# talmolab/sleap-nn

Hardware: AMD Instinct MI355X
Metric: frames/sec bottom-up UNet 1024x1024 inference (higher is better)
Workload: dtype f32

## Files before the change

sleap_nn_amd/csrc/model.hip:

```cpp
#include <algorithm>
#include <atomic>
#include <cmath>
#include <cstring>
#include <mutex>
#include <type_traits>
#include <vector>

#include "model_internal.h"
#include "train_kernels.h"

namespace ph {

static thread_local std::string g_err;

void set_error(const char* fmt, ...) {
  char buf[1024];
  va_list ap;
  va_start(ap, fmt);
  vsnprintf(buf, sizeof(buf), fmt, ap);
  va_end(ap);
  g_err = buf;
}

}
// ... 353 lines not shown
        if (!widx_ok(d.weight) || !widx_ok(d.bias)) return fail("weight index out of range", i);
        if (weight_numel[d.bias] != d.cout) return fail("bias size mismatch", i);
        if (d.kind == PH_OP_CONVT && d.ksize != 3) return fail("transposed conv: only kernel 3 (stride 2, padding 1, output padding 1)", i);
        if (d.ksize != 3) {
          if (!(d.ksize & 1) || d.ksize < 1 || d.ksize > 9) return fail("kernel_size must be odd and <= 9", i);
          if (weight_numel[d.weight] != (int64_t)(d.cin0 + d.cin1) * d.cout * d.ksize * d.ksize) return fail("weight size mismatch", i);
          const int coutp_k = pad16(d.cout);
          op.bn_g = gemm_choose_bn(coutp_k);
          auto pack_k = [&](const auto* w, auto& out) { pack_gemm(w, d.cout, d.cin0, d.cin1, d.ksize * d.ksize, op.bn_g, out); };
          ok = pack_upload(m, pack_k, weights[d.weight], index_array(d.weight), &op.w_gemm_dev) == PH_OK &&
               pack_upload(m, pad_vec((size_t)((coutp_k + op.bn_g - 1) / op.bn_g) * op.bn_g, d.cout), weights[d.bias], index_array(d.bias), &op.b_gemm_dev) == PH_OK;
          if (ok && d.kind == PH_OP_CONV) {
            const int cin_total = d.cin0 + d.cin1;
            const int parts[2] = {d.cin0, d.cin1}, offs[2] = {0, d.cin0};
            int max_bn = 32;
            const std::vector<double> iwk = index_array(d.weight);
            for (int part = 0; part < 2 && ok; ++part) {
              if (parts[part] <= 0) continue;
              op.bn_dk[part] = gemm_choose_bn(pad16(parts[part]));
              max_bn = std::max(max_bn, op.bn_dk[part]);
              auto pack_dk = [&](const auto* w, auto& out) {
                std::remove_reference_t<decltype(out)> dw;
                dgrad_weight(w, d.cout, cin_total, offs[part], parts[part], dw, d.ksize);
                pack_gemm(dw.data(), parts[part], d.cout, 0, d.ksize * d.ksize, op.bn_dk[part], out);
              };
              ok = pack_upload(m, pack_dk, weights[d.weight], iwk, &op.wdk_gemm_dev[part]) == PH_OK;
            }
            if (ok) {
              std::vector<float> zb((size_t)pad16(std::max(d.cin0, d.cin1)) + 2 * max_bn, 0.f);
              ok = upload(m, zb, &op.zero_bias_dev) == PH_OK;
            }
          }
          break;
        }
        if (d.kind == PH_OP_CONVT && d.cin1 != 0) return fail("transposed conv takes one source", i);
        if (weight_numel[d.weight] != (int64_t)(d.cin0 + d.cin1) * d.cout * 9) return fail("weight size mismatch", i);
        const int coutp = pad16(d.cout);
        op.bn = choose_bn(coutp);
        const bool tr = d.kind == PH_OP_CONVT;
        const std::vector<double> iw = index_array(d.weight), ib = index_array(d.bias);
        auto pack_reg = [&](const auto* w, auto& out) { pack_conv(w, tr, d.cin0, d.cin1, d.cout, op.bn, out); };
        auto pack_dma = [&](const auto* w, auto& out) {
          std::remove_reference_t<decltype(out)> tmp;
          pack_conv(w, tr, d.cin0, d.cin1, d.cout, op.bn, tmp);
          repack_dma(tmp, op.bn, out);
        };
        ok = pack_upload(m, pack_reg, weights[d.weight], iw, &op.w_dev) == PH_OK && pack_upload(m, pack_dma, weights[d.weight], iw, &op.w_dma_dev) == PH_OK &&
             pack_upload(m, pad_vec((size_t)((coutp + op.bn - 1) / op.bn) * op.bn, d.cout), weights[d.bias], ib, &op.b_dev) == PH_OK;
        auto derive_wino = [&](const float* src, int cin_a, int cin_b, int cout_, int bn, float** dst) {
          if (bn != 64 && bn != 32) return true;
          const int panels = ((pad16(cout_) + bn - 1) / bn) * (pad16(cin_a) / 16 + (cin_b > 0 ? pad16(cin_b) / 16 : 0));
          float* w = nullptr;
          if (hipMalloc(&w, (size_t)wino_pack_floats(panels, bn) * sizeof(float)) != hipSuccess) return false;
          m->allocs.push_back(w);
          if (launch_wino_pack(src, w, panels, bn, nullptr) != PH_OK) return false;
          add_derived(m, DERIVED_WINO, src, w, panels, bn);
          *dst = w;
          return true;
        };
        if (ok && !tr) ok = derive_wino(op.w_dev, d.cin0, d.cin1, d.cout, op.bn, &op.w_wino_dev);
        auto derive_wino2 = [&](const float* src, int cin_a, int cin_b, int cout_, int bn, float** dst) {
          if (bn != 64) return true;
          const int panels = ((pad16(cout_) + 63) / 64) * (pad16(cin_a) / 16 + (cin_b > 0 ? pad16(cin_b) / 16 : 0));
          float* w = nullptr;
          if (hipMalloc(&w, (size_t)wino2d_pack_floats(panels, 64) * sizeof(float)) != hipSuccess) return false;
          m->allocs.push_back(w);
          if (launch_wino2d_pack(src, w, panels, 64, nullptr) != PH_OK) return false;
          add_derived(m, DERIVED_WINO2D, src, w, panels, 64);
          *dst = w;
          return true;
        };
        if (ok && !tr) ok = derive_wino2(op.w_dev, d.cin0, d.cin1, d.cout, op.bn, &op.w_wino2_dev);
        if (ok && !tr && op.bn == 32 && coutp == 32 && pad16(d.cin0) + (d.cin1 > 0 ? pad16(d.cin1) : 0) >= 64) {
          auto pack_64 = [&](const auto* w, auto& out) { pack_conv(w, false, d.cin0, d.cin1, d.cout, 64, out); };
          ok = pack_upload(m, pack_64, weights[d.weight], iw, &op.w_n64_dev) == PH_OK && pack_upload(m, pad_vec(64, d.cout), weights[d.bias], ib, &op.b_n64_dev) == PH_OK &&
               derive_wino2(op.w_n64_dev, d.cin0, d.cin1, d.cout, 64, &op.w_wino2_dev);
        }
        auto derive_wino4 = [&](const float* src, int cin_a, int cin_b, int cout_, int bn, float** dst) {
          if (bn != 64 || pad16(cin_a) + (cin_b > 0 ? pad16(cin_b) : 0) < 64) return true;
          const int ntiles = (pad16(cout_) + 63) / 64, nchunks = pad16(cin_a) / 16 + (cin_b > 0 ? pad16(cin_b) / 16 : 0);
          float* w = nullptr;
          if (hipMalloc(&w, (size_t)wino4_pack_floats(ntiles, nchunks) * sizeof(float)) != hipSuccess) return false;
          m->allocs.push_back(w);
          if (launch_wino4_pack(src, w, ntiles, nchunks, nullptr) != PH_OK) return false;
          add_derived(m, DERIVED_WINO4, src, w, ntiles, nchunks);
          *dst = w;
          return true;
        };
        if (ok && !tr) ok = derive_wino4(op.w_dev, d.cin0, d.cin1, d.cout, op.bn, &op.w_wino4_dev);
        if (ok && !tr && op.w_n64_dev) ok = derive_wino4(op.w_n64_dev, d.cin0, d.cin1, d.cout, 64, &op.w_wino4_dev);
        auto derive_w16 = [&](const float* src, int cin_, int cout_, int bn, float** dst, int cin_b = 0) {
          const int cip = pad16(cin_), cibp = cin_b > 0 ? pad16(cin_b) : 0, cop = pad16(cout_);
          if (bn != 32 || !w16_shape_ok(cip, cibp, cop)) return true;
          const int chunks = (cip + cibp) / 16, nbs = cop / 16;
          float* w = nullptr;
          if (hipMalloc(&w, (size_t)w16_pack_floats(chunks, nbs) * sizeof(float)) != hipSuccess) return false;
          m->allocs.push_back(w);
          if (launch_w16_pack(src, w, chunks, nbs, nullptr) != PH_OK) return false;
          add_derived(m, DERIVED_W16, src, w, chunks, nbs);
          *dst = w;
          return true;
        };
        if (ok && !tr) ok = derive_w16(op.w_dev, d.cin0, d.cout, op.bn, &op.w_w16_dev, d.cin1);
        if (ok && !tr) {
          const int nblocks = coutp / 16, chunks16 = pad16(d.cin0) / 16 + (d.cin1 > 0 ? pad16(d.cin1) / 16 : 0);
          float* w = nullptr;
          ok = hipMalloc(&w, (size_t)sm_pack_floats(nblocks, chunks16) * sizeof(float)) == hipSuccess;
          if (ok) {
            m->allocs.push_back(w);
            ok = launch_sm_pack(op.w_dev, w, nblocks, chunks16, op.bn, nullptr) == PH_OK;
            add_derived(m, DERIVED_SMALLMAP, op.w_dev, w, nblocks, chunks16).n_tiles = op.bn;
            op.w_sm_dev = w;
          }
        }
        if (ok && !tr) {
          op.bn_g = gemm_choose_bn(coutp);
          auto pack_g = [&](const auto* w, auto& out) { pack_gemm(w, d.cout, d.cin0, d.cin1, 9, op.bn_g, out); };
          ok = pack_upload(m, pack_g, weights[d.weight], iw, &op.w_gemm_dev) == PH_OK &&
               pack_upload(m, pad_vec((size_t)((coutp + op.bn_g - 1) / op.bn_g) * op.bn_g, d.cout), weights[d.bias], ib, &op.b_gemm_dev) == PH_OK;
        }
        const bool c16 = d.kind == PH_OP_CONV && d.cin1 == 0 && d.cin0 <= 16 && d.cout <= 16;
        if (ok && c16) {
          auto pack_16 = [&](const auto* w, auto& out) { pack_c16(w, d.cout, d.cin0, out); };
          auto pack_16d = [&](const auto* w, auto& out) {
            std::remove_reference_t<decltype(out)> dw;
            dgrad_weight(w, d.cout, d.cin0, 0, d.cin0, dw);
            pack_c16(dw.data(), d.cin0, d.cout, out);
          };
          ok = pack_upload(m, pack_16, weights[d.weight], iw, &op.w16_dev) == PH_OK && pack_upload(m, pack_16d, weights[d.weight], iw, &op.wd16_dev) == PH_OK;
        }
        if (ok && tr) {
          op.bn_t = gemm_choose_bn(coutp);
          const size_t npad_t = (size_t)((coutp + op.bn_t - 1) / op.bn_t) * op.bn_t;
          for (int ph = 0; ph < 4 && ok; ++ph) {
            const int py = ph >> 1, px = ph & 1, nt = (1 + py) * (1 + px);
            auto pack_p = [&](const auto* w, auto& out) {
              std::remove_reference_t<decltype(out)> wp((size_t)d.cout * d.cin0 * nt);
              for (int t = 0; t < nt; ++t) {
                const int ty = px ? t >> 1 : t, tx = px ? t & 1 : 0;
                const int ky = py ? 2 * ty : 1, kx = px ? 2 * tx : 1;
                for (int co = 0; co < d.cout; ++co)
                  for (int ci = 0; ci < d.cin0; ++ci) wp[((size_t)co * d.cin0 + ci) * nt + t] = w[(((size_t)ci * d.cout + co) * 3 + ky) * 3 + kx];
              }
              pack_gemm(wp.data(), d.cout, d.cin0, 0, nt, op.bn_t, out);
            };
            ok = pack_upload(m, pack_p, weights[d.weight], iw, &op.wt_phase_dev[ph]) == PH_OK;
          }
          if (ok) ok = pack_upload(m, pad_vec(npad_t, d.cout), weights[d.bias], ib, &op.bt_dev) == PH_OK;
          if (ok && d.weight2 >= 0) {
            if (!widx_ok(d.weight2) || !widx_ok(d.bias2) || weight_numel[d.weight2] != d.cout || weight_numel[d.bias2] != d.cout) return fail("transposed conv: scale / shift must be (cout)", i);
            ok = pack_upload(m, pad_vec(npad_t, d.cout), weights[d.weight2], index_array(d.weight2), &op.wt_scale_dev) == PH_OK &&
                 pack_upload(m, pad_vec(npad_t, d.cout), weights[d.bias2], index_array(d.bias2), &op.wt_shift_dev) == PH_OK;
          }
          if (ok) {
            const int cinp = pad16(d.cin0);
            op.bn_td = gemm_choose_bn(cinp);
            auto pack_dg = [&](const auto* w, auto& out) { pack_gemm(w, d.cin0, d.cout, 0, 9, op.bn_td, out); };
            std::vector<float> zb((size_t)cinp + 128, 0.f);
            ok = pack_upload(m, pack_dg, weights[d.weight], iw, &op.wt_dgrad_dev) == PH_OK && upload(m, zb, &op.zero_bias_dev) == PH_OK;
          }
        }
        if (ok && d.kind == PH_OP_CONV) {
          const int cin_total = d.cin0 + d.cin1;
          const int parts[2] = {d.cin0, d.cin1}, offs[2] = {0, d.cin0};
          int max_bn = 32;
          for (int part = 0; part < 2 && ok; ++part) {
            if (parts[part] <= 0) continue;
            op.bn_d[part] = choose_bn(pad16(parts[part]));
// ... 414 lines not shown
```

sleap_nn_amd/csrc/net_kernels.h:

```cpp
#pragma once
#include <hip/hip_runtime.h>

#include <algorithm>
#include <cstdint>

namespace ph {

struct ConvArgs {
  const float* src0;
  const float* src1;
  const float* wpack;
  const float* bias;
  float* dst;
  int c0p, c1p, coutp;
  int B, H, W;
  int relu;
  int bn;
  unsigned long long* clock_probe = nullptr;
  const float* wpack_dma = nullptr;
  const float* zeros = nullptr;
  int accumulate = 0;
  int dma_stagger = 1;
  const float* wpack_wino = nullptr;
  const float* wpack_wino2 = nullptr;
// ... 143 lines not shown
  int sh = 0, sw = 0;
};
int64_t window_attn_bwd_scratch_floats(int B, int H, int W, int C, int heads, int w);
int launch_window_attn_bwd(const WindowAttnBwdArgs& a, hipStream_t s);
int launch_patch_merge_gather(const float* src, float* dst, int B, int H, int W, int c, hipStream_t s);
int launch_patch_merge_scatter(const float* gsrc, float* gdst, int accumulate, int B, int H, int W, int c, hipStream_t s);
int launch_grad_fanout(const float* gy, float* gx, int accumulate, size_t n, hipStream_t s);
int launch_scale_samples(const float* src, const float* scale, float* dst, size_t per_sample, int B, hipStream_t s);
int launch_scale_samples_add(float* dst, const float* res, const float* scale, size_t per_sample, int B, hipStream_t s);
int launch_vec_add(float* dst, const float* src, int n, hipStream_t s);
int launch_patch_merge_ln(const float* src, const float* gamma, const float* beta, float* dst, int B, int H, int W, int c, float eps, hipStream_t s);
struct WindowAttnF16Args {
  const void* qkv = nullptr;
  const float* table = nullptr;
  const float* qkv_bias = nullptr;
  void* dst = nullptr;
  int B = 0, H = 0, W = 0, C = 0, heads = 0;
  int w = 0;
  int sh = 0, sw = 0;
};
int launch_window_attn_f16(const WindowAttnF16Args& a, hipStream_t s);
int launch_patch_merge_ln_f16(const void* src, const float* gamma, const float* beta, void* dst, int B, int H, int W, int c, float eps, hipStream_t s);
int launch_gemm(const GemmArgs& a, hipStream_t s);
int launch_patch_stem_norm(const PatchStemArgs& a, hipStream_t s);
struct GrnArgs {
  const float* src = nullptr;
  const float* weight = nullptr;
  const float* bias = nullptr;
  float* dst = nullptr;
  float* partial = nullptr;
  int B = 0, HW = 0, c = 0, cp = 0;
};
int grn_slices(int HW);
int grn_slice_pixels(int HW);
int64_t grn_scratch_floats(int B, int HW, int cp);
int launch_grn(const GrnArgs& a, hipStream_t s);
int grn_fused_nseg(int HW);
int64_t grn_fused_partial_floats(int M, int HW, int cp);
int launch_grn_finalize(const float* partial, const float* weight, float* scale, int B, int HW, int c, int cp, hipStream_t s);
int launch_grn_fold_bias(const float* w2, const float* b2, const float* grn_bias, float* dst, int cout, int cin, hipStream_t s);
int64_t gemm_pack_floats(int coutp, int c0p, int bn);
int launch_grn_scale_weights(const float* wpack, const float* scale, float* dst, int B, int coutp, int c0p, int bn, hipStream_t s);
struct MlpArgs {
  const float* x = nullptr;
  const float* w1img = nullptr;
  const float* w2img = nullptr;
  const float* b1 = nullptr;
  const float* b2 = nullptr;
  const float* scale = nullptr;
  const float* residual = nullptr;
  float* dst = nullptr;
  int M = 0, C = 0;
};
bool cnblock_mlp_fits(int c, int cp, int hidden);
int launch_cnblock_mlp(const MlpArgs& a, hipStream_t s);
int gemm_choose_bn(int coutp);
int prepare_convnext_kernels();
int launch_stem(const StemArgs& a, hipStream_t s);
int prepare_kernels();
int conv_lds_bytes(int bn);
int launch_conv3x3(const ConvArgs& a, hipStream_t s);
int launch_wino_pack(const float* wpack, float* wino, int panels, int bn, hipStream_t s);
int64_t wino_pack_floats(int panels, int bn);
struct PackSegment {
  const float* src;
  float* dst;
  unsigned long long total;
  int bn;
  unsigned first_block;
};
int launch_wino_pack_multi(const PackSegment* seg_dev, int n_seg, unsigned total_blocks, hipStream_t s);
int launch_wino2d_pack_multi(const PackSegment* seg_dev, int n_seg, unsigned total_blocks, hipStream_t s);
int launch_stem_wino_pack(const float* w1, float* w1w, hipStream_t s);
int launch_stem_wino2d_pack(const float* w1, float* w2, hipStream_t s);
int launch_conv3x3_dma(const ConvArgs& a, hipStream_t s);
bool conv3x3_dma_honours_mask(const ConvArgs& a);
bool conv3x3_dma_is_f2x2(const ConvArgs& a);
bool conv3x3_dma_is_wino2d(const ConvArgs& a);
bool conv3x3_dma_is_w16_head(const ConvArgs& a);
int conv3x3_dma_variant(const ConvArgs& a);
int launch_wino2d_pack(const float* wpack, float* wino, int panels, int bn, hipStream_t s);
int64_t wino2d_pack_floats(int panels, int bn);
int launch_conv3x3_wino2d(const ConvArgs& a, hipStream_t s);
int launch_wino4_pack(const float* wpack, float* wino, int ntiles, int nchunks, hipStream_t s);
int64_t wino4_pack_floats(int ntiles, int nchunks);
int launch_conv3x3_wino4(const ConvArgs& a, hipStream_t s);
bool wino4_fits(const ConvArgs& a);
bool conv3x3_dma_is_wino4(const ConvArgs& a);
int prepare_wino4_kernels();
bool wino2d_fits(const ConvArgs& a);
int wino2d_ksplit(const ConvArgs& a);
int launch_splitk_reduce(const float* part, long long stride, int ks, const float* bias, float* dst, float* dst_pool, int B, int H, int W, int coutp, int relu, hipStream_t s);
int wino4_ksplit_shape(int B, int H, int W, int cinp, int coutp, int splitk, int n_cu);
int64_t wino4_split_scratch_bytes(int B, int H, int W, int cinp, int coutp, int splitk, int n_cu);
int wino2d_ksplit_shape(int B, int H, int W, int cinp, int coutp, int splitk, int n_cu);
int64_t wino2d_split_scratch_bytes(int B, int H, int W, int cinp, int coutp, int splitk, int n_cu);
int prepare_wino2d_kernels();
int launch_w16_pack(const float* wpack, float* w16, int chunks, int nbs, hipStream_t s);
int64_t w16_pack_floats(int chunks, int nbs);
int launch_conv3x3_w16(const ConvArgs& a, hipStream_t s);
bool w16_fits(const ConvArgs& a);
bool w16_takes_head(const ConvArgs& a);
bool w16_shape_ok(int c0p, int c1p, int coutp);
int prepare_w16_kernels();
int launch_sm_pack(const float* wpack, float* dst, int nblocks, int chunks16, int bn, hipStream_t s);
int64_t sm_pack_floats(int nblocks, int chunks16);
int launch_conv3x3_sm(const ConvArgs& a, hipStream_t s);
bool sm_fits(const ConvArgs& a);
double sm_cost_us(const ConvArgs& a, int n_cu);
bool conv3x3_takes_sm(const ConvArgs& a);
int launch_input_conv(const InputConvArgs& a, hipStream_t s);
int launch_pool(const float* src, float* dst, int B, int H, int W, int cp, hipStream_t s);
int launch_upsample(const float* src, float* dst, int B, int H, int W, int cp, hipStream_t s);
int launch_zero_stuff(const float* src, float* dst, int B, int H, int W, int cp, hipStream_t s);
int launch_global_maxpool(const float* src, float* dst, int B, int HW, int cp, hipStream_t s);
int launch_softmax_rows(float* x, int rows, int n, hipStream_t s);
int launch_nhwc_to_nchw(const float* src, float* dst, int B, int HW, int cp, int c, hipStream_t s);

}
```

sleap_nn_amd/csrc/wino4_kernels.hip:

```cpp
#include <type_traits>

#include "common.h"
#include "net_kernels.h"

#ifndef W4_EXP
#define W4_EXP 0
#endif

namespace ph {

typedef float f32x16 __attribute__((ext_vector_type(16)));
typedef float f32x4 __attribute__((ext_vector_type(4)));
typedef float f32x2 __attribute__((ext_vector_type(2)));

constexpr int W4_TX = 8, W4_TY = 4;
constexpr int W4_PW = 4 * W4_TX;
constexpr int W4_PH = 4 * W4_TY;
constexpr int W4_RAW_PITCH = 36;
constexpr int W4_RAW_PLANE = 688;
constexpr int W4_RAW_FLOATS = 3072;
static_assert(W4_RAW_PITCH >= W4_PW + 2 && W4_RAW_PITCH % 4 == 0, "a halo row fits its pitch and starts 16-byte aligned");
static_assert(W4_RAW_PLANE >= (W4_PH + 3) * W4_RAW_PITCH && W4_RAW_PLANE % 64 % 32 == 16, "a plane holds 18 halo rows + the overshoot row; planes 16 banks apart (mod 32): conflict-free ds_read_b128");
static_assert(4 * W4_RAW_PLANE <= W4_RAW_FLOATS, "four planes fit a raw slot");
constexpr int W4_V_FLOATS = 36 * 128;
constexpr int W4_LDS_FLOATS = 36 * 1024;
constexpr int W4_Q_FLOATS = 36 * 64 * 4;
constexpr int P4_WAVE_FLOATS = 4 * 256 + 128;

__device__ __forceinline__ float wino4_g_row(int k, float g0, float g1, float g2) {
  switch (k) {
    case 0: return 0.25f * g0;
    case 1: return (-1.f / 6.f) * ((g0 + g2) + g1);
    case 2: return (-1.f / 6.f) * ((g0 + g2) - g1);
    case 3: return (1.f / 24.f) * g0 + ((1.f / 12.f) * g1 + (1.f / 6.f) * g2);
    case 4: return (1.f / 24.f) * g0 + ((-1.f / 12.f) * g1 + (1.f / 6.f) * g2);
    default: return g2;
  }
}
__global__ __launch_bounds__(256) void wino4_pack_kernel(const float* __restrict__ src, float* __restrict__ dst, int ntiles, int nchunks) {
  __shared__ float unit[W4_Q_FLOATS];
  const int quarter = blockIdx.x % (4 * nchunks), ntile = blockIdx.x / (4 * nchunks);
  const int tid = threadIdx.x;
  const int row = tid >> 2, kcl = tid & 3;
  const int nt = row >> 5, lx = row & 31, lh = kcl >> 1, j = kcl & 1;
  const float* w = src + (((size_t)ntile * nchunks + (quarter >> 2)) * 9 * 64 + row) * 16 + (quarter & 3) * 4 + kcl;
  const size_t ts = (size_t)64 * 16;
  float g[9];
#pragma unroll
  for (int t = 0; t < 9; ++t) g[t] = w[t * ts];
#pragma unroll
  for (int xi = 0; xi < 6; ++xi) {
    float h[3];
#pragma unroll
    for (int kx = 0; kx < 3; ++kx) h[kx] = wino4_g_row(xi, g[0 * 3 + kx], g[1 * 3 + kx], g[2 * 3 + kx]);
#pragma unroll
    for (int nu = 0; nu < 6; ++nu) {
      const float u = wino4_g_row(nu, h[0], h[1], h[2]);
      const int p = xi * 6 + nu, pgp = p / 9, pl = p % 9;
      unit[(nt * 4 + pgp) * P4_WAVE_FLOATS + (pl < 8 ? (((pl >> 1) * 64 + lh * 32 + lx) << 2) + j * 2 + (pl & 1) : 1024 + ((lh * 32 + lx) << 1) + j)] = u;
    }
  }
  __syncthreads();
  float* out = dst + (size_t)blockIdx.x * W4_Q_FLOATS;
#pragma unroll 4
  for (int i = tid; i < W4_Q_FLOATS; i += 256) out[i] = unit[i];
}
int64_t wino4_pack_floats(int ntiles, int nchunks) { return (int64_t)ntiles * 4 * nchunks * W4_Q_FLOATS; }
int launch_wino4_pack(const float* wpack, float* wino, int ntiles, int nchunks, hipStream_t s) {
  hipLaunchKernelGGL(wino4_pack_kernel, dim3((unsigned)(ntiles * 4 * nchunks)), dim3(256), 0, s, wpack, wino, ntiles, nchunks);
  PH_HIP_CHECK(hipGetLastError());
  return PH_OK;
}

__device__ __forceinline__ void w4_deal_tile(int id, int tiles, int nt_count, int rot, int* tile, int* ntile) {
  if ((tiles & 7) == 0) {
    const int xcd = id & 7, j = id >> 3;
    *ntile = (j % nt_count + rot) % nt_count;
    *tile = xcd * (tiles >> 3) + j / nt_count;
  } else {
    *ntile = (id % nt_count + rot) % nt_count;
    *tile = id / nt_count;
  }
}

__device__ __forceinline__ void w4_col_pass(const float (&t)[6], float (&v)[6]) {
  const float a = fmaf(-4.f, t[2], t[4]);
  const float b = fmaf(-4.f, t[1], t[3]);
  const float c = t[4] - t[2];
  const float d0 = t[3] - t[1];
  const float d = d0 + d0;
  v[0] = fmaf(4.f, t[0], fmaf(-5.f, t[2], t[4]));
  v[1] = a + b;
  v[2] = a - b;
  v[3] = c + d;
  v[4] = c - d;
  v[5] = fmaf(4.f, t[1], fmaf(-5.f, t[3], t[5]));
}

template <int P, int N>
__device__ __forceinline__ void p4_vput(float* slot, int vwq, int vwd, const float* v) {
  if constexpr (N > 0) {
    constexpr int pgc = P / 9, pl = P % 9;
    if constexpr (pl == 8) {
      slot[pgc * P4_WAVE_FLOATS + vwd] = v[0];
      p4_vput<P + 1, N - 1>(slot, vwq, vwd, v + 1);
    } else if constexpr ((pl & 1) == 0 && N >= 2) {
      *reinterpret_cast<float2*>(slot + pgc * P4_WAVE_FLOATS + (pl >> 1) * 256 + vwq) = make_float2(v[0], v[1]);
      p4_vput<P + 2, N - 2>(slot, vwq, vwd, v + 2);
    } else {
      slot[pgc * P4_WAVE_FLOATS + (pl >> 1) * 256 + vwq + (pl & 1)] = v[0];
      p4_vput<P + 1, N - 1>(slot, vwq, vwd, v + 1);
    }
  }
}

template <bool LOWRES, bool KS = false>
__global__ __launch_bounds__(512) void conv3x3_wino4_kernel(ConvArgs a) {
  extern __shared__ __attribute__((aligned(16))) float lds[];
  const int tid = threadIdx.x;
  const int lane = tid & 63;
  const int pw = __builtin_amdgcn_readfirstlane(tid >> 6);
  const int nt = pw >> 2, pg = pw & 3;
  const int lx = lane & 31, lh = lane >> 5;
  const int xg = pw < 4 ? (pw >> 1) : 2 + ((pw - 4) >> 1);
  const int typ = 2 * (pw & 1) + (lane >> 5), txp = (lane >> 2) & 7, cp = lane & 3;

  const int tiles_x = (a.W + W4_PW - 1) / W4_PW;
  const int tiles_y = (a.H + W4_PH - 1) / W4_PH;
  const int tiles = tiles_x * tiles_y * a.B;
  const int ntc = (a.coutp + 63) / 64;
  const int units = tiles * ntc;
  const int total = KS ? units * a.ksplit : units;
  const int Q0 = a.c0p / 4, Q1 = a.c1p / 4, Q = Q0 + Q1;
  constexpr int lowres = LOWRES ? 1 : 0;
  const int Hl = a.H >> 1, Wl = a.W >> 1;

#ifdef W4_CLOCK
  const unsigned long long clk_c0 = __builtin_amdgcn_s_memtime(), clk_r0 = __builtin_amdgcn_s_memrealtime();
#endif
  float* const rawbuf = lds;
  float* const vbuf = lds + 2 * W4_RAW_FLOATS;

  const float alpha = xg == 0 ? -4.f : -1.f, beta = xg == 0 ? 1.f : 2.f, nbeta = -beta;
  const int pbase_f = cp * W4_RAW_PLANE + (4 * typ + (xg == 2 ? 0 : 1)) * W4_RAW_PITCH + 4 * txp;
  const int pbase_l = cp * W4_RAW_PLANE + (2 * typ) * W4_RAW_PITCH + 2 * txp;
  const int lhy = (pw * 64 + lane) / (W4_PW + 2), lhx = (pw * 64 + lane) - lhy * (W4_PW + 2);
  const int lwr = lhy * W4_RAW_PITCH + lhx;
  const int vwq = ((cp >> 1) * 32 + typ * 8 + txp) * 4 + (cp & 1) * 2;
  const int vwd = 1024 + ((cp >> 1) * 32 + typ * 8 + txp) * 2 + (cp & 1);
  const int vrq = pg * P4_WAVE_FLOATS + lane * 4, vrd = pg * P4_WAVE_FLOATS + 1024 + lane * 2;

  struct Plan {
    int b, x0, y0, ntile;
  };
  const int G = (int)gridDim.x;
  const bool rotate = (a.coutp & 63) != 0 && (a.coutp & 63) <= 32 && ntc > 1 && (((tiles & 7) == 0) ? ((G & 7) == 0 && (G >> 3) % ntc == 0) : (G % ntc == 0));
  auto setup = [&](int vid, Plan& P) {
    int t, ntile;
    w4_deal_tile(vid, tiles, ntc, rotate ? vid / G : 0, &t, &ntile);
    const int tx = t % tiles_x;
    t /= tiles_x;
    const int ty = t % tiles_y;
    P.b = t / tiles_y;
    P.x0 = tx * W4_PW;
    P.y0 = ty * W4_PH;
    P.ntile = ntile;
  };

  const __amdgpu_buffer_rsrc_t wrsrc = __builtin_amdgcn_make_buffer_rsrc((void*)a.wpack_wino4, 0, (int)((unsigned)ntc * (unsigned)Q * (unsigned)(W4_Q_FLOATS * 4)), 0x00020000);
  const unsigned w_lane = (unsigned)(pw * P4_WAVE_FLOATS + lane * 4) * 4u;
  const unsigned w_lane9 = (unsigned)(pw * P4_WAVE_FLOATS + 1024 + lane * 2) * 4u;

  for (int vid = blockIdx.x; vid < total; vid += gridDim.x) {
#ifdef W4_STAMP
    const unsigned long long tile_t0 = __builtin_amdgcn_s_memtime();
#endif
    Plan P;
    const int ksl = KS ? vid / units : 0;
    const int qbeg = KS ? ksl * Q / a.ksplit : 0;
    const int qend = KS ? (ksl + 1) * Q / a.ksplit : Q;
    setup(KS ? vid - ksl * units : vid, P);
    unsigned off0[2], off1[2];
#pragma unroll
    for (int i = 0; i < 2; ++i) {
      const int hy = lhy + 15 * i, hx = lhx;
      const int gy = P.y0 + hy - 1, gx = P.x0 + hx - 1;
      const bool in = (i == 0 || pw < 2) && hy < W4_PH + 2 && gy >= 0 && gy < a.H && gx >= 0 && gx < a.W;
      off0[i] = in ? (unsigned)((P.b * a.H + gy) * a.W + gx) * (unsigned)(a.c0p * 4) : 0xFFFFFF00u;
      if (!lowres) {
        off1[i] = (in && a.c1p > 0) ? (unsigned)((P.b * a.H + gy) * a.W + gx) * (unsigned)(a.c1p * 4) : 0xFFFFFF00u;
      } else {
        const int sy = min(max((P.y0 >> 1) - 1 + hy, 0), Hl - 1), sx = min(max((P.x0 >> 1) - 1 + hx, 0), Wl - 1);
        off1[i] = (hy < W4_PH / 2 + 2 && hx < W4_PW / 2 + 2) ? (unsigned)((P.b * Hl + sy) * Wl + sx) * (unsigned)(a.c1p * 4) : 0xFFFFFF00u;
      }
    }
    const __amdgpu_buffer_rsrc_t rsrc0 = __builtin_amdgcn_make_buffer_rsrc((void*)a.src0, 0, (int)((unsigned)(a.B * a.H * a.W) * (unsigned)(a.c0p * 4)), 0x00020000);
// ... 269 lines not shown
        P4_SB
        P4_ST(1)
        if constexpr (MM) {
          acc[8] = P4_MFMA(wf9[0], vf9.x, acc[8]);
          vf0 = *reinterpret_cast<const f32x4*>(vq);
          acc[6] = P4_MFMA(wf[3][2], vf3[2], acc[6]);
        }
        P4_SB
        load_raw(q + 3);
        P4_SB
        P4_ST(2)
        if constexpr (MM) {
          acc[7] = P4_MFMA(wf[3][3], vf3[3], acc[7]);
          load_w(q, 3);
          vf1 = *reinterpret_cast<const f32x4*>(vq + 256);
          P4_ST(3)
          acc[8] = P4_MFMA(wf9[1], vf9.y, acc[8]);
          load_w(q, 4);
        }
        t_rows(xg_tag, lr_tag, 0);
        t_read(xg_tag, lr_tag, raw, 1);
        P4_SB
        P4_ST(4)
        if constexpr (MM) {
          acc[0] = P4_MFMA(wf[0][0], vf0[0], acc[0]);
          acc[1] = P4_MFMA(wf[0][1], vf0[1], acc[1]);
          vf2 = *reinterpret_cast<const f32x4*>(vq + 512);
          acc[0] = P4_MFMA(wf[0][2], vf0[2], acc[0]);
          acc[1] = P4_MFMA(wf[0][3], vf0[3], acc[1]);
          load_w(q + 1, 0);
        }
        t_rows(xg_tag, lr_tag, 1);
        P4_SB
        P4_ST(5)
        if constexpr (MM) {
          acc[2] = P4_MFMA(wf[1][0], vf1[0], acc[2]);
          acc[3] = P4_MFMA(wf[1][1], vf1[1], acc[3]);
          vf3 = *reinterpret_cast<const f32x4*>(vq + 768);
        }
        t_cols(xg_tag, lr_tag, first, vslot);
        if constexpr (MM) {
          acc[2] = P4_MFMA(wf[1][2], vf1[2], acc[2]);
          acc[3] = P4_MFMA(wf[1][3], vf1[3], acc[3]);
          load_w(q + 1, 1);
        }
        P4_SB
        P4_ST(6)
        if constexpr (MM) {
          acc[4] = P4_MFMA(wf[2][0], vf2[0], acc[4]);
          acc[5] = P4_MFMA(wf[2][1], vf2[1], acc[5]);
          vf9 = *reinterpret_cast<const float2*>(vd);
        }
        if constexpr (PAIR) t_cols(xg_tag, lr_tag, second, vslot);
        if constexpr (MM) {
          acc[4] = P4_MFMA(wf[2][2], vf2[2], acc[4]);
          acc[5] = P4_MFMA(wf[2][3], vf2[3], acc[5]);
          load_w(q + 1, 2);
        }
        P4_SB
        P4_ST(7)
        asm volatile("s_waitcnt lgkmcnt(0)" ::: "memory");
        if (!(W4_EXP & 4)) __builtin_amdgcn_s_barrier();
        P4_SB
        P4_ST_END
      }
    };
    auto run = [&](auto xg_tag, auto mm_tag) __attribute__((always_inline)) {
      if constexpr (LOWRES) {
        const int qs = min(max(Q0 - 1, qbeg), qend);
        quarters(xg_tag, mm_tag, std::false_type{}, qbeg, qs);
        quarters(xg_tag, mm_tag, std::true_type{}, qs, qend);
      } else {
        quarters(xg_tag, mm_tag, std::false_type{}, qbeg, qend);
      }
    };
    auto run_mm = [&](auto mm_tag) __attribute__((always_inline)) {
      switch (xg) {
        case 0: run(std::integral_constant<int, 0>{}, mm_tag); break;
        case 1: run(std::integral_constant<int, 1>{}, mm_tag); break;
        case 2: run(std::integral_constant<int, 2>{}, mm_tag); break;
        default: run(std::integral_constant<int, 3>{}, mm_tag); break;
      }
    };
    if (nt == 1 && P.ntile * 64 + 32 >= a.coutp) {
      run_mm(std::false_type{});
    } else {
      run_mm(std::true_type{});
      acc[6] = P4_MFMA(wf[3][0], vf3[0], acc[6]);
      acc[7] = P4_MFMA(wf[3][1], vf3[1], acc[7]);
      acc[8] = P4_MFMA(wf9[0], vf9.x, acc[8]);
      acc[6] = P4_MFMA(wf[3][2], vf3[2], acc[6]);
      acc[7] = P4_MFMA(wf[3][3], vf3[3], acc[7]);
      acc[8] = P4_MFMA(wf9[1], vf9.y, acc[8]);
    }

#ifdef W4_STAMP
    const unsigned long long tile_t2 = __builtin_amdgcn_s_memtime();
#endif
    float* const exch = lds;
    auto dump = [&](int r) __attribute__((always_inline)) {
      int d0 = ((pg * 9 * 32 + lx) * 8 + ((nt * 4 + lh) ^ (lx & 7))) << 2;
      asm volatile("" : "+v"(d0));
#pragma unroll
      for (int kk = 0; kk < 2; ++kk) {
        float* const dk = exch + (d0 ^ (kk << 3));
#pragma unroll
        for (int i = 0; i < 9; ++i) {
          f32x4 v;
          if (r == 0) {
            v[0] = acc[i][4 * kk + 0];
            v[1] = acc[i][4 * kk + 1];
            v[2] = acc[i][4 * kk + 2];
            v[3] = acc[i][4 * kk + 3];
          } else {
            v[0] = acc[i][8 + 4 * kk + 0];
            v[1] = acc[i][8 + 4 * kk + 1];
            v[2] = acc[i][8 + 4 * kk + 2];
            v[3] = acc[i][8 + 4 * kk + 3];
          }
          *reinterpret_cast<f32x4*>(dk + i * 1024) = v;
        }
      }
      asm volatile("s_waitcnt lgkmcnt(0)" ::: "memory");
    };
    auto finish = [&](int round) __attribute__((always_inline)) {
      const int tile = tid >> 4, cq = (tid >> 1) & 7, hc = tid & 1;
      const int ty = tile >> 3, tx = tile & 7;
      int z0 = ((tile * 8 + (cq ^ (tile & 7))) << 2) + 2 * hc;
      asm volatile("" : "+v"(z0));
      const float* zp = exch + z0;
      f32x2 z[4][6];
#pragma unroll
      for (int n = 0; n < 6; ++n) {
        f32x2 m[6];
#pragma unroll
        for (int x = 0; x < 6; ++x) m[x] = *reinterpret_cast<const f32x2*>(zp + (x * 6 + n) * 1024);
#pragma unroll
        for (int e = 0; e < 2; ++e) {
          const float s12 = m[1][e] + m[2][e], d12 = m[1][e] - m[2][e], s34 = m[3][e] + m[4][e], d34 = m[3][e] - m[4][e];
          z[0][n][e] = (m[0][e] + s12) + s34;
          z[1][n][e] = fmaf(2.f, d34, d12);
          z[2][n][e] = fmaf(4.f, s34, s12);
          z[3][n][e] = fmaf(8.f, d34, d12) + m[5][e];
        }
      }
      const int co = P.ntile * 64 + (cq >> 2) * 32 + round * 16 + (cq & 3) * 4 + 2 * hc;
      const f32x2 bias = KS ? f32x2{0.f, 0.f} : *reinterpret_cast<const f32x2*>(a.bias + co);
      const int oy0 = P.y0 + 4 * ty, ox = P.x0 + 4 * tx;
      const bool live = oy0 < a.H && ox < a.W && co < a.coutp;
      f32x2 prow[2];
#pragma unroll
      for (int aa = 0; aa < 4; ++aa) {
        const f32x2 s12 = z[aa][1] + z[aa][2], d12 = z[aa][1] - z[aa][2], s34 = z[aa][3] + z[aa][4], d34 = z[aa][3] - z[aa][4];
        f32x2 y[4];
        y[0] = ((z[aa][0] + s12) + s34) + bias;
        y[1] = (d12 + 2.f * d34) + bias;
        y[2] = (s12 + 4.f * s34) + bias;
        y[3] = ((d12 + 8.f * d34) + z[aa][5]) + bias;
        if (live) {
          float* const dp = a.dst + ((size_t)(P.b * a.H + oy0 + aa) * a.W + ox) * a.coutp + co + (KS ? (size_t)ksl * a.split_stride : (size_t)0);
#pragma unroll
          for (int bb = 0; bb < 4; ++bb) {
            f32x2 v = y[bb];
            if (a.relu) {
#pragma unroll
              for (int e = 0; e < 2; ++e) v[e] = fmaxf(v[e], 0.f);
            }
            if (a.relu_mask_src) {
              const f32x2 f = *reinterpret_cast<const f32x2*>(a.relu_mask_src + (dp - a.dst) + (size_t)bb * a.coutp);
#pragma unroll
              for (int e = 0; e < 2; ++e) v[e] = f[e] > 0.f ? v[e] : 0.f;
            }
            y[bb] = v;
            if ((KS || !a.skip_dst) && !(W4_EXP & 512)) *reinterpret_cast<f32x2*>(dp + (size_t)bb * a.coutp) = v;
          }
          if (!KS && a.dst_pool) {
            f32x2 m0, m1;
#pragma unroll
            for (int e = 0; e < 2; ++e) {
              m0[e] = fmaxf(y[0][e], y[1][e]);
              m1[e] = fmaxf(y[2][e], y[3][e]);
            }
            if (aa & 1) {
#pragma unroll
              for (int e = 0; e < 2; ++e) {
                m0[e] = fmaxf(m0[e], prow[0][e]);
                m1[e] = fmaxf(m1[e], prow[1][e]);
              }
              float* const pp = a.dst_pool + ((size_t)(P.b * (a.H >> 1) + ((oy0 + aa) >> 1)) * (a.W >> 1) + (ox >> 1)) * a.coutp + co;
              *reinterpret_cast<f32x2*>(pp) = m0;
              *reinterpret_cast<f32x2*>(pp + a.coutp) = m1;
            } else {
              prow[0] = m0;
              prow[1] = m1;
            }
          }
        }
      }
      asm volatile("s_waitcnt lgkmcnt(0)" ::: "memory");
    };
#ifdef W4_STAMP
    unsigned long long e1 = 0, e2 = 0, e3 = 0;
#define P4_ET(x) x = __builtin_amdgcn_s_memtime();
#else
#define P4_ET(x)
#endif
    dump(0);
    __builtin_amdgcn_s_barrier();
    P4_ET(e1)
    finish(0);
    __builtin_amdgcn_s_barrier();
    P4_ET(e2)
    dump(1);
    __builtin_amdgcn_s_barrier();
    P4_ET(e3)
    finish(1);
    __builtin_amdgcn_s_barrier();
#ifdef W4_STAMP
    if (a.clock_probe && lane == 0 && vid == (int)blockIdx.x) {
      unsigned long long* o = a.clock_probe + ((size_t)blockIdx.x * 12 + pw) * 8;
#ifdef W4_STTILE
      o[0] = (tile_t1 - tile_t0) * (unsigned long long)(qend - qbeg);
      o[1] = st[0] + st[1] + st[2] + st[3] + st[4] + st[5] + st[6] + st[7];
      o[2] = (e1 - tile_t2) * (unsigned long long)(qend - qbeg);
      o[3] = (e2 - e1) * (unsigned long long)(qend - qbeg);
      o[4] = (e3 - e2) * (unsigned long long)(qend - qbeg);
      o[5] = (__builtin_amdgcn_s_memtime() - e3) * (unsigned long long)(qend - qbeg);
      o[6] = o[7] = 0;
#else
#pragma unroll
      for (int i = 0; i < 8; ++i) o[i] = st[i];
#endif
    }
#endif
  }
#ifdef W4_CLOCK
  if (a.clock_probe && tid == 0) {
    a.clock_probe[blockIdx.x * 2] = __builtin_amdgcn_s_memtime() - clk_c0;
    a.clock_probe[blockIdx.x * 2 + 1] = __builtin_amdgcn_s_memrealtime() - clk_r0;
  }
#endif
}

int prepare_wino4_kernels() {
  hipError_t e = hipSuccess;
  if (e == hipSuccess) e = hipFuncSetAttribute(reinterpret_cast<const void*>(conv3x3_wino4_kernel<false, false>), hipFuncAttributeMaxDynamicSharedMemorySize, W4_LDS_FLOATS * (int)sizeof(float));
  if (e == hipSuccess) e = hipFuncSetAttribute(reinterpret_cast<const void*>(conv3x3_wino4_kernel<true, false>), hipFuncAttributeMaxDynamicSharedMemorySize, W4_LDS_FLOATS * (int)sizeof(float));
  if (e == hipSuccess) e = hipFuncSetAttribute(reinterpret_cast<const void*>(conv3x3_wino4_kernel<false, true>), hipFuncAttributeMaxDynamicSharedMemorySize, W4_LDS_FLOATS * (int)sizeof(float));
  if (e == hipSuccess) e = hipFuncSetAttribute(reinterpret_cast<const void*>(conv3x3_wino4_kernel<true, true>), hipFuncAttributeMaxDynamicSharedMemorySize, W4_LDS_FLOATS * (int)sizeof(float));
  if (e != hipSuccess) {
    set_error("hipFuncSetAttribute(wino4) failed: %s", hipGetErrorString(e));
    return PH_E_HIP;
  }
  return PH_OK;
}

bool wino4_fits(const ConvArgs& a) {
  if (!a.wpack_wino4 || a.bn != 64 || (a.H & 3) || (a.W & 3) || a.head_w || a.accumulate) return false;
  if (a.src1_lowres && (!a.src1 || (a.H & 1) || (a.W & 1))) return false;
  const uint64_t px = (uint64_t)a.B * a.H * a.W;
  if (px * (uint64_t)a.c0p * 4 >= 0xFFFFFF00ull || px * (uint64_t)a.c1p * 4 >= 0xFFFFFF00ull || px >= 0x7FFFFFFFull) return false;
  const uint64_t wbytes = (uint64_t)((a.coutp + 63) / 64) * (uint64_t)((a.c0p + a.c1p) / 4) * W4_Q_FLOATS * 4;
  if (wbytes >= 0xFFFFFF00ull) return false;
  if (a.use_wino4 >= 2) return true;
  int n_cu = 0;
  if (device_cu_count(&n_cu) != PH_OK || n_cu <= 0) n_cu = 256;
  const bool may_split = a.split_scratch != nullptr;
  const int ks4 = may_split ? wino4_ksplit_shape(a.B, a.H, a.W, a.c0p + a.c1p, a.coutp, a.splitk, n_cu) : 1;
  const int ks2 = may_split ? wino2d_ksplit_shape(a.B, a.H, a.W, a.c0p + a.c1p, a.coutp, a.splitk, n_cu) : 1;
  const long ntc = (a.coutp + 63) / 64;
  const long t4 = (long)((a.H + W4_PH - 1) / W4_PH) * ((a.W + W4_PW - 1) / W4_PW) * a.B * ntc;
  const long t2 = (long)((a.H + 15) / 16) * ((a.W + 15) / 16) * a.B * ntc;
  const double Qn = (a.c0p + a.c1p) / 4.0;
  const double cost4 = (double)((t4 * ks4 + n_cu - 1) / n_cu) * (11.0 + 1.5 * Qn / ks4) + (ks4 > 1 ? 8.0 : 0.0);
  const double cost2 = (double)((t2 * ks2 + n_cu - 1) / n_cu) * (8.0 + 1.0 * Qn / ks2) + (ks2 > 1 ? 8.0 : 0.0);
  return cost4 <= cost2;
}
// ... 56 lines not shown
```

Before: 3036.

## Widen wino4 epilogue stores to 16 bytes via DPP lane pair trade

The Winograd F(4,3) epilogue used to write 8-byte float2 values per output pixel. Adjacent lanes now swap halves with DPP cndmask, so each lane holds four channels for one pixel and issues 16-byte stores with an sc1 cache policy. Pooled outputs get the same treatment. To keep channels contiguous, the weight pack and the channel mapping change for full tiles, and ReLU is hoisted ahead of the trade. This adds inline-asm DPP work, and the weight layout and epilogue mapping must stay consistent.

```diff
diff --git a/sleap_nn_amd/csrc/model.hip b/sleap_nn_amd/csrc/model.hip
--- a/sleap_nn_amd/csrc/model.hip
+++ b/sleap_nn_amd/csrc/model.hip
@@ -459,8 +459,8 @@
           float* w = nullptr;
           if (hipMalloc(&w, (size_t)wino4_pack_floats(ntiles, nchunks) * sizeof(float)) != hipSuccess) return false;
           m->allocs.push_back(w);
-          if (launch_wino4_pack(src, w, ntiles, nchunks, nullptr) != PH_OK) return false;
-          add_derived(m, DERIVED_WINO4, src, w, ntiles, nchunks);
+          if (launch_wino4_pack(src, w, pad16(cout_), nchunks, nullptr) != PH_OK) return false;
+          add_derived(m, DERIVED_WINO4, src, w, pad16(cout_), nchunks);
           *dst = w;
           return true;
         };
diff --git a/sleap_nn_amd/csrc/net_kernels.h b/sleap_nn_amd/csrc/net_kernels.h
--- a/sleap_nn_amd/csrc/net_kernels.h
+++ b/sleap_nn_amd/csrc/net_kernels.h
@@ -249,7 +249,7 @@
 int launch_wino2d_pack(const float* wpack, float* wino, int panels, int bn, hipStream_t s);
 int64_t wino2d_pack_floats(int panels, int bn);
 int launch_conv3x3_wino2d(const ConvArgs& a, hipStream_t s);
-int launch_wino4_pack(const float* wpack, float* wino, int ntiles, int nchunks, hipStream_t s);
+int launch_wino4_pack(const float* wpack, float* wino, int coutp, int nchunks, hipStream_t s);
 int64_t wino4_pack_floats(int ntiles, int nchunks);
 int launch_conv3x3_wino4(const ConvArgs& a, hipStream_t s);
 bool wino4_fits(const ConvArgs& a);
diff --git a/sleap_nn_amd/csrc/wino4_kernels.hip b/sleap_nn_amd/csrc/wino4_kernels.hip
--- a/sleap_nn_amd/csrc/wino4_kernels.hip
+++ b/sleap_nn_amd/csrc/wino4_kernels.hip
@@ -5,6 +5,9 @@
 
 #ifndef W4_EXP
 #define W4_EXP 0
+#endif
+#ifndef W4_ST_POLICY
+#define W4_ST_POLICY 2
 #endif
 
 namespace ph {
@@ -27,6 +30,7 @@
 constexpr int W4_Q_FLOATS = 36 * 64 * 4;
 constexpr int P4_WAVE_FLOATS = 4 * 256 + 128;
 
+__host__ __device__ __forceinline__ bool w4_tile_in_halves(int coutp, int ntile) { return ntile * 64 + 32 >= coutp; }
 __device__ __forceinline__ float wino4_g_row(int k, float g0, float g1, float g2) {
   switch (k) {
     case 0: return 0.25f * g0;
@@ -37,12 +41,13 @@
     default: return g2;
   }
 }
-__global__ __launch_bounds__(256) void wino4_pack_kernel(const float* __restrict__ src, float* __restrict__ dst, int ntiles, int nchunks) {
+__global__ __launch_bounds__(256) void wino4_pack_kernel(const float* __restrict__ src, float* __restrict__ dst, int ntiles, int nchunks, int half_last) {
   __shared__ float unit[W4_Q_FLOATS];
   const int quarter = blockIdx.x % (4 * nchunks), ntile = blockIdx.x / (4 * nchunks);
   const int tid = threadIdx.x;
   const int row = tid >> 2, kcl = tid & 3;
-  const int nt = row >> 5, lx = row & 31, lh = kcl >> 1, j = kcl & 1;
+  const bool halves = half_last && ntile == ntiles - 1;
+  const int nt = halves ? row >> 5 : (row >> 4) & 1, lx = halves ? row & 31 : (row & 15) + 16 * (row >> 5), lh = kcl >> 1, j = kcl & 1;
   const float* w = src + (((size_t)ntile * nchunks + (quarter >> 2)) * 9 * 64 + row) * 16 + (quarter & 3) * 4 + kcl;
   const size_t ts = (size_t)64 * 16;
   float g[9];
@@ -66,8 +71,9 @@
   for (int i = tid; i < W4_Q_FLOATS; i += 256) out[i] = unit[i];
 }
 int64_t wino4_pack_floats(int ntiles, int nchunks) { return (int64_t)ntiles * 4 * nchunks * W4_Q_FLOATS; }
-int launch_wino4_pack(const float* wpack, float* wino, int ntiles, int nchunks, hipStream_t s) {
-  hipLaunchKernelGGL(wino4_pack_kernel, dim3((unsigned)(ntiles * 4 * nchunks)), dim3(256), 0, s, wpack, wino, ntiles, nchunks);
+int launch_wino4_pack(const float* wpack, float* wino, int coutp, int nchunks, hipStream_t s) {
+  const int ntiles = (coutp + 63) / 64;
+  hipLaunchKernelGGL(wino4_pack_kernel, dim3((unsigned)(ntiles * 4 * nchunks)), dim3(256), 0, s, wpack, wino, ntiles, nchunks, w4_tile_in_halves(coutp, ntiles - 1) ? 1 : 0);
   PH_HIP_CHECK(hipGetLastError());
   return PH_OK;
 }
@@ -112,6 +118,35 @@
       p4_vput<P + 1, N - 1>(slot, vwq, vwd, v + 1);
     }
   }
+}
+
+__device__ __forceinline__ f32x4 w4_pair_trade(f32x2 lo, f32x2 hi) {
+  float o0, o1, o2, o3;
+  asm volatile(
+      "s_nop 1\n\t"
+      "s_mov_b32 vcc_lo, 0x55555555\n\t"
+      "s_mov_b32 vcc_hi, 0x55555555\n\t"
+      "v_cndmask_b32_dpp %0, %6, %4, vcc quad_perm:[1,0,3,2] row_mask:0xf bank_mask:0xf\n\t"
+      "v_cndmask_b32_dpp %1, %7, %5, vcc quad_perm:[1,0,3,2] row_mask:0xf bank_mask:0xf\n\t"
+      "s_mov_b32 vcc_lo, 0xaaaaaaaa\n\t"
+      "s_mov_b32 vcc_hi, 0xaaaaaaaa\n\t"
+      "v_cndmask_b32_dpp %2, %4, %6, vcc quad_perm:[1,0,3,2] row_mask:0xf bank_mask:0xf\n\t"
+      "v_cndmask_b32_dpp %3, %5, %7, vcc quad_perm:[1,0,3,2] row_mask:0xf bank_mask:0xf"
+      : "=&v"(o0), "=&v"(o1), "=&v"(o2), "=&v"(o3)
+      : "v"(lo[0]), "v"(lo[1]), "v"(hi[0]), "v"(hi[1])
+      : "vcc");
+  return f32x4{o0, o1, o2, o3};
+}
+__device__ __forceinline__ void w4_store16(float* p, f32x4 v) {
+#if W4_ST_POLICY == 1
+  __builtin_nontemporal_store(v, reinterpret_cast<f32x4*>(p));
+#elif W4_ST_POLICY == 2
+  asm volatile("global_store_dwordx4 %0, %1, off sc1\n\ts_nop 0" ::"v"(p), "v"(v) : "memory");
+#elif W4_ST_POLICY == 3
+  asm volatile("global_store_dwordx4 %0, %1, off sc0 sc1\n\ts_nop 0" ::"v"(p), "v"(v) : "memory");
+#else
+  *reinterpret_cast<f32x4*>(p) = v;
+#endif
 }
 
 template <bool LOWRES, bool KS = false>
@@ -547,7 +582,7 @@
         default: run(std::integral_constant<int, 3>{}, mm_tag); break;
       }
     };
-    if (nt == 1 && P.ntile * 64 + 32 >= a.coutp) {
+    if (nt == 1 && w4_tile_in_halves(a.coutp, P.ntile)) {
       run_mm(std::false_type{});
     } else {
       run_mm(std::true_type{});
@@ -589,10 +624,12 @@
       asm volatile("s_waitcnt lgkmcnt(0)" ::: "memory");
     };
     auto finish = [&](int round) __attribute__((always_inline)) {
-      const int tile = tid >> 4, cq = (tid >> 1) & 7, hc = tid & 1;
+      const int tile = tid >> 4, cq = (tid >> 1) & 7;
+      int hc = tid & 1;
       const int ty = tile >> 3, tx = tile & 7;
       int z0 = ((tile * 8 + (cq ^ (tile & 7))) << 2) + 2 * hc;
       asm volatile("" : "+v"(z0));
+      asm volatile("" : "+v"(hc));
       const float* zp = exch + z0;
       f32x2 z[4][6];
 #pragma unroll
@@ -609,11 +646,11 @@
           z[3][n][e] = fmaf(8.f, d34, d12) + m[5][e];
         }
       }
-      const int co = P.ntile * 64 + (cq >> 2) * 32 + round * 16 + (cq & 3) * 4 + 2 * hc;
-      const f32x2 bias = KS ? f32x2{0.f, 0.f} : *reinterpret_cast<const f32x2*>(a.bias + co);
+      const int co = P.ntile * 64 + (cq & 3) * 4 + (w4_tile_in_halves(a.coutp, P.ntile) ? (cq >> 2) * 32 + round * 16 : round * 32 + (cq >> 2) * 16);
+      const f32x2 bias = KS ? f32x2{0.f, 0.f} : *reinterpret_cast<const f32x2*>(a.bias + co + 2 * hc);
       const int oy0 = P.y0 + 4 * ty, ox = P.x0 + 4 * tx;
       const bool live = oy0 < a.H && ox < a.W && co < a.coutp;
-      f32x2 prow[2];
+      f32x4 prow;
 #pragma unroll
       for (int aa = 0; aa < 4; ++aa) {
         const f32x2 s12 = z[aa][1] + z[aa][2], d12 = z[aa][1] - z[aa][2], s34 = z[aa][3] + z[aa][4], d34 = z[aa][3] - z[aa][4];
@@ -622,42 +659,38 @@
         y[1] = (d12 + 2.f * d34) + bias;
         y[2] = (s12 + 4.f * s34) + bias;
         y[3] = ((d12 + 8.f * d34) + z[aa][5]) + bias;
+        if (a.relu) {
+#pragma unroll
+          for (int bb = 0; bb < 4; ++bb) {
+#pragma unroll
+            for (int e = 0; e < 2; ++e) y[bb][e] = fmaxf(y[bb][e], 0.f);
+          }
+        }
+        const f32x4 o0 = w4_pair_trade(y[0], y[2]), o1 = w4_pair_trade(y[1], y[3]);
+        f32x4 o[2] = {o0, o1};
         if (live) {
-          float* const dp = a.dst + ((size_t)(P.b * a.H + oy0 + aa) * a.W + ox) * a.coutp + co + (KS ? (size_t)ksl * a.split_stride : (size_t)0);
-#pragma unroll
-          for (int bb = 0; bb < 4; ++bb) {
-            f32x2 v = y[bb];
-            if (a.relu) {
-#pragma unroll
-              for (int e = 0; e < 2; ++e) v[e] = fmaxf(v[e], 0.f);
+          float* const dp = a.dst + ((size_t)(P.b * a.H + oy0 + aa) * a.W + ox + 2 * hc) * a.coutp + co + (KS ? (size_t)ksl * a.split_stride : (size_t)0);
+#pragma unroll
+          for (int c = 0; c < 2; ++c) {
+            f32x4 v = o[c];
+            if (a.relu_mask_src) {
+              const f32x4 f = *reinterpret_cast<const f32x4*>(a.relu_mask_src + (dp - a.dst) + (size_t)c * a.coutp);
+#pragma unroll
+              for (int e = 0; e < 4; ++e) v[e] = f[e] > 0.f ? v[e] : 0.f;
             }
-            if (a.relu_mask_src) {
-              const f32x2 f = *reinterpret_cast<const f32x2*>(a.relu_mask_src + (dp - a.dst) + (size_t)bb * a.coutp);
-#pragma unroll
-              for (int e = 0; e < 2; ++e) v[e] = f[e] > 0.f ? v[e] : 0.f;
-            }
-            y[bb] = v;
-            if ((KS || !a.skip_dst) && !(W4_EXP & 512)) *reinterpret_cast<f32x2*>(dp + (size_t)bb * a.coutp) = v;
+            o[c] = v;
+            if ((KS || !a.skip_dst) && !(W4_EXP & 512)) w4_store16(dp + (size_t)c * a.coutp, v);
           }
           if (!KS && a.dst_pool) {
-            f32x2 m0, m1;
-#pragma unroll
-            for (int e = 0; e < 2; ++e) {
-              m0[e] = fmaxf(y[0][e], y[1][e]);
-              m1[e] = fmaxf(y[2][e], y[3][e]);
-            }
+            f32x4 m;
+#pragma unroll
+            for (int e = 0; e < 4; ++e) m[e] = fmaxf(o[0][e], o[1][e]);
             if (aa & 1) {
 #pragma unroll
-              for (int e = 0; e < 2; ++e) {
-                m0[e] = fmaxf(m0[e], prow[0][e]);
-                m1[e] = fmaxf(m1[e], prow[1][e]);
-              }
-              float* const pp = a.dst_pool + ((size_t)(P.b * (a.H >> 1) + ((oy0 + aa) >> 1)) * (a.W >> 1) + (ox >> 1)) * a.coutp + co;
-              *reinterpret_cast<f32x2*>(pp) = m0;
-              *reinterpret_cast<f32x2*>(pp + a.coutp) = m1;
+              for (int e = 0; e < 4; ++e) m[e] = fmaxf(m[e], prow[e]);
+              w4_store16(a.dst_pool + ((size_t)(P.b * (a.H >> 1) + ((oy0 + aa) >> 1)) * (a.W >> 1) + (ox >> 1) + hc) * a.coutp + co, m);
             } else {
-              prow[0] = m0;
-              prow[1] = m1;
+              prow = m;
             }
           }
         }
```

New measurement: 3084 (median of 6 runs). 1.02x the previous value.
